# acids-ircam/RAVE

Measured on NVIDIA H100. Metric: audio-seconds/s (v2 train step fwd+bwd, 48 kHz), higher is better.
Workload: dtype bf16

## Files before the change

### include/rave_b200.h

```cpp
#ifndef RAVE_B200_H
#define RAVE_B200_H

#include <stddef.h>
#include <stdint.h>

#ifdef __cplusplus
extern "C" {
#endif

#define RAVE_ACT_NONE 0
#define RAVE_ACT_LEAKY 1
#define RAVE_ACT_SNAKE 2

#define RAVE_PREC_FP32 0
#define RAVE_PREC_BF16 1
#define RAVE_PREC_TF32 2

int rave_b200_version(void);
const char *rave_b200_last_error(void);
unsigned long long rave_b200_launch_count(void);

int rave_pqmf_analysis_fwd(const float *x, const float *taps, float *y, int B, int T, int Lout,
                           int ntaps, int pad_l, int flip_sign, void *stream);
int rave_pqmf_synthesis_fwd(const float *x, const float *w, float *out, int B, int L, int K,
                            int pad_l, float scale, int flip_sign, void *stream);
int rave_pqmf_analysis_fast(const float *x, const float *Ct, const float *Qt, float *y, int B, int T, int Lout,
                            int pad_l, int flip_sign, void *stream);
int rave_pqmf_synthesis_fast(const float *x, const float *Cc, const float *Qt, float *out, int B, int L,
                             int pad_l, float scale, int flip_sign, void *stream);

int rave_conv1d_gather_f32(const float *src, const float *w, const float *bias, const float *res,
                           float *out, int B, int Cs, int Ls, int Cm, int Lo, int K, int stride,
                           int dil, int pad_l, long ws_m, long ws_c, int act, float slope,
                           const float *alpha, int post_act, float post_slope, const float *post_x,
                           const float *post_alpha, void *stream);
int rave_conv1d_scatter_f32(const float *src, const float *w, const float *bias, const float *res,
                            float *out, int B, int Cs, int Ls, int Cm, int Lo, int K, int stride,
                            int dil, int pad_l, long ws_m, long ws_c, int act, float slope,
                            const float *alpha, int post_act, float post_slope, const float *post_x,
                            const float *post_alpha, void *stream);

size_t rave_conv1d_wgrad_workspace_bytes(int B, int Ca, int Cc, int Lp, int K);
int rave_conv1d_wgrad_f32(const float *P, const float *Q, float *dw, int B, int Ca, int Lp, int Cc,
                          int Lq, int K, int stride, int dil, int pad_l, long os_a, long os_c,
                          int act_p, int act_q, float slope, const float *alpha, void *workspace,
                          void *stream);

int rave_weight_norm_fwd(const float *v, const float *g, float *w, float *norm_out, int C0, int R,
                         void *stream);
int rave_weight_norm_bwd(const float *dw, const float *v, const float *g, const float *norm,
                         float *dv, float *dg, int C0, int R, void *stream);

int rave_act_fwd(const float *x, float *y, int B, int C, int L, int act, float slope,
                 const float *alpha, void *stream);
int rave_act_bwd(const float *dy, const float *x, float *dx, float *dalpha, int B, int C, int L,
                 int act, float slope, const float *alpha, void *stream);
int rave_am_tanh_fwd(const float *x, float *y, int B, int C, int L, void *stream);
int rave_am_tanh_bwd(const float *dy, const float *x, float *dx, int B, int C, int L, void *stream);
int rave_reparam_fwd(const float *z, const float *eps, float *zs, float *kl_sum, int B, int C, int L, void *stream);
int rave_mmd_fwd(const float *z, const float *prior, float *means, float *mmd, int B, int D, int L, void *stream);
int rave_mmd_bwd(const float *z, const float *prior, const float *g, float *dz, int B, int D, int L, void *stream);
int rave_sphere_norm_fwd(const float *z, float *out, float *norm, int B, int C, int L, void *stream);
int  rave_latent_moments(const float *z, int B, int C, int L, int D, double *state, double *work, void *stream);
long rave_latent_moments_workspace_bytes(int B, int L, int D);
int rave_sphere_norm_bwd(const float *g, const float *out, const float *norm, float *dz, int B, int C, int L,
                         void *stream);

int rave_conv1d_tc_supported(int Cin, int Cout, int K, int stride, int dil);
int rave_dilated_unit_tc_supported(int C, int L);
int rave_dilated_unit_tc_fwd(const void *xa_bf16, const void *w3t_bf16, const void *w1t_bf16, void *a1_out,
                             float *out_f32, void *out_act, int B, int C, int L, int pitch, int dil, int pad_l,
                             float slope_in, float slope_mid, int act_out, float slope_out, void *stream);
int rave_conv1d_tc_plan(int B, int Cin, int Cout, int Lout, int K);
int rave_conv1d_tc_pp_stages(int B, int Cin, int Cout, int Lout, int K, int fm, int res_bf16);
int rave_conv1d_tc_pp_fwd_stages(int B, int Cin, int Cout, int Lout, int K);
int rave_conv1d_tc_wide_stages(int B, int Cin, int Cout, int Lout, int K);
int rave_conv1d_tc_fwd(const void *xa_bf16, const void *wt_bf16, const float *bias, const float *res,
                       const void *res_bf16, const void *dact_src_bf16, const void *res_act_bf16, float res_slope,
                       float *out_f32, void *out_act_bf16,
                       int B, int Cin, int Lin, int in_pitch, int Cout, int Lout,
                       int K, int stride, int dil, int pad_l, int act, float slope, int out_rows,
                       int out_row_stride, int out_row_offset, const float *fm_d, int fm_bh, void *stream);
int rave_conv1d_tc_fwd_x3(const void *xa_bf16, const void *wt_bf16, const float *bias, const float *res,
                          const void *res_act, float res_slope, float *out_f32, void *out_act, int B, int Cin, int Lin,
                          int in_pitch, int Cout, int Lout, int K, int stride, int dil, int pad_l, int act, float slope,
                          int out_rows, int out_row_stride, int out_row_offset, int act_cs, void *stream);
int rave_conv1d_tc_wgrad_splits(int B, int Cm, int Lp, int Cn, int K);
int rave_conv1d_tc_wgrad_plan(int B, int Cm, int Lp, int Cn, int K);
int rave_time_stack_cl(const float *x, void *out_bf16, int B, int C, int T, int F, int Fp, int Cp, int kt, int pt,
                       void *stream);
int rave_time_stack_cl_bwd(const void *g_bf16, float *gx, int B, int C, int T, int F, int Fp, int Cp, int kt, int pt,
                           void *stream);
int rave_time_stack_nhwc(const float *x, void *out_bf16, int B, int C, int T, int F, long sb, long st, int Fp, int Cp, int kt,
                         int pt, void *stream);
int rave_time_stack_nhwc_bwd(const void *g_bf16, float *gx, int B, int C, int T, int F, int Fp, int Cp, int kt, int pt,
                             void *stream);
int rave_time_stack_nhwc_dil(const float *x, void *out_bf16, int B, int C, int T, int F, long sb, long st, int Fp, int Cp,
                             int kt, int pt, int dil, void *stream);
int rave_time_stack_nhwc_dil_bwd(const void *g_bf16, float *gx, int B, int C, int T, int F, int Fp, int Cp, int kt, int pt,
                                 int dil, void *stream);
int rave_l1_stats_f32(const float *t, const float *v, float *stats, long n, void *stream);
int rave_l1_grad_f32(const float *t, const float *v, const float *d, float *gt, float *gv, long n, void *stream);
int rave_leaky_fm_fwd(const float *x, float *a, float *stats, long H, float slope, void *stream);
int rave_leaky_fm_bwd(const float *a, const float *g, const float *d, float *gx, long H, float slope, void *stream);
int rave_leaky_fm_stack_fwd(const float *x, float *a, float *stats, void *xs_bf16, long Rh, int T, int F, int C, int Fp,
                            float slope, void *stream);
int rave_leaky_fm_stack_bwd(const float *a, const void *gxs_bf16, const float *ga, const float *d, float *gx, long Rh, int T,
                            int F, int C, int Fp, float slope, void *stream);
int rave_leaky_fm_stack_dil_fwd(const float *x, float *a, float *stats, void *xs_bf16, long Rh, int T, int F, int C, int Fp,
                                int dil, float slope, void *stream);
int rave_leaky_fm_stack_dil_bwd(const float *a, const void *gxs_bf16, const float *ga, const float *d, float *gx, long Rh,
                                int T, int F, int C, int Fp, int dil, float slope, void *stream);
int rave_snake_cl_fwd(const void *h_bf16, const float *alpha, void *a_bf16, long rows, int C, void *stream);
int rave_snake_cl_bwd(const void *ga_bf16, const void *h_bf16, const float *alpha, const void *add_bf16, void *gh_bf16,
                      float *dalpha, long rows, int C, void *stream);
int rave_adain_cl_stats(const void *h_bf16, int B, int L, int pitch, int C, float *mean_x, float *std_x, float *mean_y,
                        float *std_y, const float *learn_x, const float *learn_y, float *num_update_x,
                        float *num_update_y, int max_batch, float *scale, float *shift, void *stream);
int rave_adain_snake_cl_fwd(void *h_bf16, const float *alpha, const float *scale, const float *shift, void *a_bf16,
                            int B, int L, int pitch, int C, void *stream);
int rave_conv1d_tc_wgrad(const void *P_bf16, const void *Q_bf16, float *dwt, float *dbias, int B, int Cm, int Lp,
                         int p_pitch, int Cn, int Lq, int q_pitch, int K, int stride, int dil, int pad_l,
                         void *stream);
int rave_tapmajor_to_weight_f32(const float *dwt, float *dw, int Cm, int Cn, int K, int transpose, int splits,
                                void *stream);
int rave_conv1d_c1_fwd(const float *x, const float *w, const float *bias, float *out_f32, void *out_act_bf16,
                       int R, int x_pitch, int Lin, int Cout, int Lout, int out_pitch, int K, int stride,
                       int pad_l, int act, float slope, void *stream);
int rave_conv1d_c1_wgrad_splits(int R, int Lout);
// ... 116 lines not shown
```

### rave_b200/_lib.py

```python
import ctypes
import os
from ctypes import c_float, c_int, c_long, c_longlong, c_size_t, c_ulonglong, c_void_p, c_char_p

_HERE = os.path.dirname(os.path.abspath(__file__))
LIB_PATH = os.path.join(_HERE, "csrc", "librave_b200.so")

_P, _I, _F, _L = c_void_p, c_int, c_float, c_long

SIGNATURES = {
    "rave_b200_version": (c_int, []),
    "rave_b200_last_error": (c_char_p, []),
    "rave_b200_launch_count": (c_ulonglong, []),
    "rave_pqmf_analysis_fwd": (c_int, [_P, _P, _P, _I, _I, _I, _I, _I, _I, _P]),
    "rave_pqmf_synthesis_fwd": (c_int, [_P, _P, _P, _I, _I, _I, _I, _F, _I, _P]),
    "rave_pqmf_analysis_fast": (c_int, [_P, _P, _P, _P, _I, _I, _I, _I, _I, _P]),
    "rave_pqmf_synthesis_fast": (c_int, [_P, _P, _P, _P, _I, _I, _I, _F, _I, _P]),
    "rave_conv1d_gather_f32": (c_int, [_P, _P, _P, _P, _P, _I, _I, _I, _I, _I, _I, _I, _I, _I, _L, _L,
                                       _I, _F, _P, _I, _F, _P, _P, _P]),
    "rave_conv1d_scatter_f32": (c_int, [_P, _P, _P, _P, _P, _I, _I, _I, _I, _I, _I, _I, _I, _I, _L, _L,
                                        _I, _F, _P, _I, _F, _P, _P, _P]),
    "rave_conv1d_wgrad_workspace_bytes": (c_size_t, [_I, _I, _I, _I, _I]),
    "rave_conv1d_wgrad_f32": (c_int, [_P, _P, _P, _I, _I, _I, _I, _I, _I, _I, _I, _I, _L, _L, _I, _I,
                                      _F, _P, _P, _P]),
    "rave_weight_norm_fwd": (c_int, [_P, _P, _P, _P, _I, _I, _P]),
    "rave_weight_norm_bwd": (c_int, [_P, _P, _P, _P, _P, _P, _I, _I, _P]),
    "rave_act_fwd": (c_int, [_P, _P, _I, _I, _I, _I, _F, _P, _P]),
    "rave_act_bwd": (c_int, [_P, _P, _P, _P, _I, _I, _I, _I, _F, _P, _P]),
    "rave_am_tanh_fwd": (c_int, [_P, _P, _I, _I, _I, _P]),
    "rave_am_tanh_bwd": (c_int, [_P, _P, _P, _I, _I, _I, _P]),
    "rave_reparam_fwd": (c_int, [_P, _P, _P, _P, _I, _I, _I, _P]),
    "rave_mmd_fwd": (c_int, [_P, _P, _P, _P, _I, _I, _I, _P]),
    "rave_mmd_bwd": (c_int, [_P, _P, _P, _P, _I, _I, _I, _P]),
    "rave_sphere_norm_fwd": (c_int, [_P, _P, _P, _I, _I, _I, _P]),
    "rave_sphere_norm_bwd": (c_int, [_P, _P, _P, _P, _I, _I, _I, _P]),
    "rave_latent_moments": (c_int, [_P, _I, _I, _I, _I, _P, _P, _P]),
    "rave_latent_moments_workspace_bytes": (c_long, [_I, _I, _I]),
    "rave_conv1d_tc_supported": (c_int, [_I, _I, _I, _I, _I]),
    "rave_dilated_unit_tc_supported": (c_int, [_I, _I]),
    "rave_dilated_unit_tc_fwd": (c_int, [_P, _P, _P, _P, _P, _P, _I, _I, _I, _I, _I, _I, _F, _F, _I, _F, _P]),
    "rave_conv1d_tc_plan": (c_int, [_I, _I, _I, _I, _I]),
    "rave_conv1d_tc_pp_stages": (c_int, [_I, _I, _I, _I, _I, _I, _I]),
    "rave_conv1d_tc_pp_fwd_stages": (c_int, [_I, _I, _I, _I, _I]),
    "rave_conv1d_tc_wide_stages": (c_int, [_I, _I, _I, _I, _I]),
    "rave_conv1d_tc_fwd": (c_int, [_P, _P, _P, _P, _P, _P, _P, _F, _P, _P, _I, _I, _I, _I, _I, _I, _I, _I, _I, _I, _I,
                                   _F, _I, _I, _I, _P, _I, _P]),
    "rave_conv1d_tc_fwd_x3": (c_int, [_P, _P, _P, _P, _P, _F, _P, _P, _I, _I, _I, _I, _I, _I, _I, _I, _I, _I, _I, _F, _I,
                                      _I, _I, _I, _P]),
    "rave_weight_prep_tc_multi_x3": (c_int, [_I, _P, _P]),
    "rave_ncl_to_cl_x3": (c_int, [_P, _P, _I, _I, _I, _P]),
    "rave_conv1d_tc_wgrad": (c_int, [_P, _P, _P, _P, _I, _I, _I, _I, _I, _I, _I, _I, _I, _I, _I, _P]),
    "rave_tapmajor_to_weight_f32": (c_int, [_P, _P, _I, _I, _I, _I, _I, _P]),
    "rave_conv1d_tc_wgrad_splits": (c_int, [_I, _I, _I, _I, _I]),
    "rave_conv1d_tc_wgrad_plan": (c_int, [_I, _I, _I, _I, _I]),
    "rave_time_stack_cl": (c_int, [_P, _P, _I, _I, _I, _I, _I, _I, _I, _I, _P]),
    "rave_time_stack_cl_bwd": (c_int, [_P, _P, _I, _I, _I, _I, _I, _I, _I, _I, _P]),
    "rave_time_stack_nhwc": (c_int, [_P, _P, _I, _I, _I, _I, ctypes.c_long, ctypes.c_long, _I, _I, _I, _I, _P]),
    "rave_time_stack_nhwc_bwd": (c_int, [_P, _P, _I, _I, _I, _I, _I, _I, _I, _I, _P]),
    "rave_time_stack_nhwc_dil": (c_int, [_P, _P, _I, _I, _I, _I, ctypes.c_long, ctypes.c_long, _I, _I, _I, _I, _I, _P]),
    "rave_time_stack_nhwc_dil_bwd": (c_int, [_P, _P, _I, _I, _I, _I, _I, _I, _I, _I, _I, _P]),
    "rave_l1_stats_f32": (c_int, [_P, _P, _P, ctypes.c_long, _P]),
    "rave_leaky_fm_fwd": (c_int, [_P, _P, _P, ctypes.c_long, ctypes.c_float, _P]),
    "rave_leaky_fm_bwd": (c_int, [_P, _P, _P, _P, ctypes.c_long, ctypes.c_float, _P]),
    "rave_leaky_fm_stack_fwd": (c_int, [_P, _P, _P, _P, ctypes.c_long, _I, _I, _I, _I, ctypes.c_float, _P]),
    "rave_leaky_fm_stack_bwd": (c_int, [_P, _P, _P, _P, _P, ctypes.c_long, _I, _I, _I, _I, ctypes.c_float, _P]),
    "rave_leaky_fm_stack_dil_fwd": (c_int, [_P, _P, _P, _P, ctypes.c_long, _I, _I, _I, _I, _I, ctypes.c_float, _P]),
    "rave_leaky_fm_stack_dil_bwd": (c_int, [_P, _P, _P, _P, _P, ctypes.c_long, _I, _I, _I, _I, _I, ctypes.c_float, _P]),
    "rave_l1_grad_f32": (c_int, [_P, _P, _P, _P, _P, ctypes.c_long, _P]),
    "rave_snake_cl_fwd": (c_int, [_P, _P, _P, ctypes.c_long, _I, _P]),
    "rave_snake_cl_bwd": (c_int, [_P, _P, _P, _P, _P, _P, ctypes.c_long, _I, _P]),
    "rave_adain_cl_stats": (c_int, [_P, _I, _I, _I, _I, _P, _P, _P, _P, _P, _P, _P, _P, _I, _P, _P, _P]),
    "rave_adain_snake_cl_fwd": (c_int, [_P, _P, _P, _P, _P, _I, _I, _I, _I, _P]),
    "rave_weight_prep_tc": (c_int, [_P, _P, _P, _P, _P, _I, _P, _P, _I, _I, _I, _I, _I, _I, _P]),
    "rave_weight_norm_bwd_tapmajor": (c_int, [_P, _P, _P, _P, _P, _P, _I, _I, _I, _I, _I, _I, _P]),
    "rave_conv1d_c1_fwd": (c_int, [_P, _P, _P, _P, _P, _I, _I, _I, _I, _I, _I, _I, _I, _I, _I, _F, _P]),
    "rave_conv1d_c1_wgrad_splits": (c_int, [_I, _I]),
    "rave_conv1d_c1_wgrad": (c_int, [_P, _P, _P, _I, _I, _I, _I, _I, _I, _I, _I, _I, _I, _P]),
    "rave_conv1d_c1_dgrad": (c_int, [_P, _P, _P, _I, _I, _I, _I, _I, _I, _I, _I, _I, _I, _P]),
    "rave_colsum_bf16": (c_int, [_P, _P, _I, _I, _I, _I, _I, _P]),
    "rave_im2col_c1": (c_int, [_P, _P, _I, _I, _I, _I, _I, _I, _I, _I, _I, _I, _I, _P]),
    "rave_gather_c1": (c_int, [_P, _P, _I, _I, _I, _I, _I, _I, _I, _I, _I, _I, _I, _P]),
    "rave_im2col_cin": (c_int, [_P, _P, _I, _I, _I, _I, _I, _I, _I, _I, _I, _I, _I, _I, _I, _P]),
    "rave_gather_cin": (c_int, [_P, _P, _I, _I, _I, _I, _I, _I, _I, _I, _I, _I, _I, _I, _I, _P]),
    "rave_fm_stats": (c_int, [_P, _P, _I, _I, _I, _I, _F, _P]),
    "rave_fm_grad": (c_int, [_P, _P, _P, _I, _I, _I, _I, _F, _P]),
    "rave_score_stats": (c_int, [_P, _P, _I, _I, _I, _I, _P]),
    "rave_score_grad": (c_int, [_P, _P, _P, _I, _I, _I, _I, _P]),
    "rave_spectral_stats": (c_int, [_P, _P, _P, _L, _F, _P]),
    "rave_spectral_grad": (c_int, [_P, _P, _P, _P, _P, _L, _F, _P]),
    "rave_stft_frames": (c_int, [_P, _P, _P, _I, _I, _I, _I, _P]),
    "rave_stft_frames_bwd": (c_int, [_P, _P, _P, _I, _I, _I, _I, _P]),
    "rave_stft_frames_valid": (c_int, [_P, _P, _P, _I, _I, _I, _I, _F, _P]),
    "rave_stft_frames_valid_bwd": (c_int, [_P, _P, _P, _I, _I, _I, _I, _F, _P]),
    "rave_rfft_bwd_scale": (c_int, [_P, _P, _L, _I, _I, _L, _L, _L, _P]),
    "rave_mel_log1p_fwd": (c_int, [_P, _P, _P, _P, _I, _I, _I, _I, _I, _F, _P]),
    "rave_mel_log1p_bwd": (c_int, [_P, _P, _P, _P, _P, _I, _I, _I, _I, _I, _F, _P]),
    "rave_gru_fwd": (c_int, [_P, _P, _P, _P, _P, _I, _I, _I, _P]),
# ... 107 lines not shown
```

### rave_b200/csrc/conv_tc.cu

```cuda
#include <string.h>

#include <type_traits>

#include "common.cuh"
#include "tc_common.cuh"

namespace rave {
namespace tc {

constexpr int BLOCK_M = 128;
constexpr int NUM_THREADS = 288;
constexpr int SMEM_MAX = 227 * 1024;

struct TcParams {
  int B, Cin, Lin, Cout, Lout, K, stride, dil, pad_l;
  int BL, BB;
  int n_lt, n_bg, n_nt;
  int num_kb;
  int act;
  float slope;
  const float *bias;
  const float *res;
  const __nv_bfloat16 *res_bf16;
  const __nv_bfloat16 *dact_src;
// ... 371 lines not shown
    for (int tile = blockIdx.x; tile < num_tiles; tile += gridDim.x, ++it) {
      const int prev = mma_mainloop<BLOCK_N, BLOCK_K, X3>(d, smem_base, ring, kblocks, lane);
      mma_drain<BLOCK_N>(d, ring, prev, lane);
      const int buf = p.nacc == 2 ? (it & 1) : 0;
      const uint32_t use = p.nacc == 2 ? (it >> 1) : it;
      mbar_wait(&tempty_bar[buf], (use & 1) ^ 1);
      acc_store<BLOCK_N>(d, threadIdx.x, 0, 128 * buf);
      mbar_arrive(&tfull_bar[buf]);
    }
  } else {
    constexpr int BOXC = L::OUT_BOXC;
    const int quad = warp & 3;
    const int row = quad * 32 + lane;
    const bool issuer = threadIdx.x == 160;
    int it = 0;
    for (int tile = blockIdx.x; tile < num_tiles; tile += gridDim.x, ++it) {
      const TileCoord t = tile_coord<BLOCK_N>(tile, p);
      const int n0 = t.n0;
      const int b = t.b0 + row / p.BL;
      const int l = t.l0 + row % p.BL;
      const bool valid = (b < p.B) && (l < p.Lout);
      const size_t orow = (size_t)b * p.out_rows + (size_t)l * p.out_row_stride + p.out_row_offset;

      const int buf = p.nacc == 2 ? (it & 1) : 0;
      const uint32_t use = p.nacc == 2 ? (it >> 1) : it;
      if (stg) {
        if (issuer) bulk_wait_read<0>();
        named_bar_sync(1, 128);
      }
      mbar_wait(&tfull_bar[buf], use & 1);
      const uint32_t taddr = (uint32_t)(128 * buf + quad * 32) << 16;
      tc_epilogue<BLOCK_N, X3, BOXC>(p, taddr, n0, valid, orow, p.fm_d ? (b < p.fm_bh ? 1 : -1) : 0, stg, row);
      __syncwarp();
      if (lane == 0) mbar_arrive(&tempty_bar[buf]);
      if (stg) {
        fence_proxy_async();
        named_bar_sync(1, 128);
        if (issuer) {
#pragma unroll
          for (int c = 0; c < BLOCK_N; c += BOXC)
            tma_store_3d(&tmap_o, stg + (c / BOXC) * (BLOCK_M * L::OUT_SPAN), n0 + c, t.l0, t.b0);
          bulk_commit();
        }
      }
    }
    if (stg && issuer) bulk_wait_all();
  }
}

constexpr int PP_THREADS = 384;

enum PpEpi : int { PP_FM = 1, PP_RS = 2, PP_FWD = 4, PP_BIAS = 8, PP_LEAKY = 16 };

template <int BLOCK_N, int BOXC, bool FM, bool RS>
__device__ __forceinline__ void pp_epilogue(float (*d)[BLOCK_N / 2], uint8_t *slot, const TcParams &p, int w, int lane,
                                            int b0) {
  constexpr int TILE_BYTES = BLOCK_M * BLOCK_N * 2;
  uint8_t *part = slot + TILE_BYTES;
  uint8_t *skip = slot + (FM ? 2 : 1) * TILE_BYTES;
  constexpr int SPAN = BOXC * 2, JB = BOXC / 8;
  const float d0 = FM ? __ldg(p.fm_d) : 0.f, d1 = FM ? __ldg(p.fm_d + 1) : 0.f;
  const uint32_t base = stg_offset<BOXC>(16 * w + (lane >> 2), 0) + 4 * (lane & 3);
#pragma unroll
  for (int h = 0; h < 2; ++h) {
#pragma unroll
    for (int r = 0; r < 2; ++r) {
      const int row = 64 * h + 16 * w + (lane >> 2) + 8 * r;
      const float d1r = (FM && b0 + row / p.BL < p.fm_bh) ? d1 : 0.f;
#pragma unroll
      for (int j = 0; j < BLOCK_N / 8; ++j) {
        const uint32_t off = (base ^ (uint32_t)((j % JB) << 4)) + (j / JB) * (BLOCK_M * SPAN) + (64 * h + 8 * r) * SPAN;
        float v0 = d[h][4 * j + 2 * r], v1 = d[h][4 * j + 2 * r + 1];
        const uint32_t dm = *reinterpret_cast<const uint32_t *>(slot + off);
        lrelu_mask(v0, v1, dm, p.slope);
        if (FM) fm_grad(v0, v1, dm, *reinterpret_cast<const uint32_t *>(part + off), d0, d1r);
        if (RS) add_bf16_pair(v0, v1, *reinterpret_cast<const uint32_t *>(skip + off));
        __nv_bfloat162 o = __floats2bfloat162_rn(v0, v1);
        *reinterpret_cast<uint32_t *>(slot + off) = *reinterpret_cast<uint32_t *>(&o);
      }
    }
  }
}

template <int BLOCK_N, int BOXC, bool BIAS, bool LEAKY, int NH = 2>
__device__ __forceinline__ void pp_fwd_epilogue(float (*d)[BLOCK_N / 2], uint8_t *slot, const TcParams &p, int w,
                                                int lane, int n0, int h0 = 0) {
  constexpr int SPAN = BOXC * 2, JB = BOXC / 8;
  const uint32_t base = stg_offset<BOXC>(16 * w + (lane >> 2), 0) + 4 * (lane & 3);
  const uint32_t sslot = smem_u32(slot);
  const float2 *bias = reinterpret_cast<const float2 *>(p.bias + n0 + 2 * (lane & 3));
#pragma unroll
  for (int j = 0; j < BLOCK_N / 8; ++j) {
    const float2 bb = BIAS ? __ldg(bias + 4 * j) : make_float2(0.f, 0.f);
    const uint32_t col = (base ^ (uint32_t)((j % JB) << 4)) + (j / JB) * (BLOCK_M * SPAN);
#pragma unroll
    for (int h = 0; h < NH; ++h) {
#pragma unroll
      for (int r = 0; r < 2; ++r) {
        float v0 = d[h][4 * j + 2 * r], v1 = d[h][4 * j + 2 * r + 1];
        if (BIAS) {
          v0 += bb.x;
          v1 += bb.y;
        }
        if (LEAKY) {
          v0 = fmaxf(v0, v0 * p.slope);
          v1 = fmaxf(v1, v1 * p.slope);
        }
        __nv_bfloat162 o = __floats2bfloat162_rn(v0, v1);
        asm volatile("st.shared.b32 [%0], %1;" ::"r"(sslot + col + (64 * (h0 + h) + 8 * r) * SPAN),
                     "r"(*reinterpret_cast<uint32_t *>(&o))
                     : "memory");
      }
    }
  }
}

template <int BLOCK_N, int BLOCK_K, int E>
__device__ __forceinline__ void conv_tc_pp_body(const CUtensorMap *tmap_a, const CUtensorMap *tmap_b,
                                                const CUtensorMap *tmap_m, const CUtensorMap *tmap_p,
                                                const CUtensorMap *tmap_r, const CUtensorMap *tmap_o,
                                                const TcParams &p) {
  using L = SmemLayout<BLOCK_N, BLOCK_K, false>;
  constexpr int BOXC = L::OUT_BOXC;
  constexpr int BOX_BYTES = BLOCK_M * L::OUT_SPAN;
// ... 169 lines not shown
      mbar_init(&empty_bar[s], 8);
    }
    mbar_init(oempty_bar, 1);
    fence_barrier_init();
  }
  __syncthreads();
  griddep_launch_dependents();
  griddep_wait();

  Ring ring{full_bar, empty_bar, STAGES, 0, 0};
  if (wg == 0) {
    warpgroup_reg_dealloc<56>();
    if (warp != 0) return;
    for (int tile = blockIdx.x; tile < num_tiles; tile += gridDim.x) {
      const TileCoord t = tile_coord<BLOCK_N>(tile, p);
      for (int k = 0; k < p.K; ++k) {
        const TapOrigin o = tap_origin(k, p.dil, p.pad_l, p.stride);
        for (int kb = 0; kb < p.num_kb; ++kb)
          produce_kblock<BLOCK_N, BLOCK_K, false>(smem, ring, &tmap_a, &tmap_b, p, t, o, k, kb);
      }
    }
  } else {
    warpgroup_reg_alloc<224>();
    const int h = wg - 1;
    const int w = warp & 3;
    const bool issuer = threadIdx.x == 128;
    const uint32_t smem_base = smem_u32(smem);
    uint8_t *slot = smem + p.ops_off;
    float d[1][BLOCK_N / 2];
    int u = 0;
    for (int tile = blockIdx.x; tile < num_tiles; tile += gridDim.x, ++u) {
      const int prev = mma_mainloop<BLOCK_N, BLOCK_K, false, 1>(d, smem_base, ring, kblocks, lane, h);
      mma_drain<BLOCK_N, 1>(d, ring, prev, lane);
      const TileCoord t = tile_coord<BLOCK_N>(tile, p);
      if (issuer && u > 0) {
        bulk_wait_read<0>();
        mbar_arrive(oempty_bar);
      }
      mbar_wait(oempty_bar, (u & 1) ^ 1);
      pp_fwd_epilogue<BLOCK_N, BOXC, BIAS, LEAKY, 1>(d, slot, p, w, lane, t.n0, h);
      fence_proxy_async();
      named_bar_sync(1, 256);
      if (issuer) {
#pragma unroll
        for (int cb = 0; cb < BLOCK_N / BOXC; ++cb)
          tma_store_3d(&tmap_o, slot + cb * BOX_BYTES, t.n0 + cb * BOXC, t.l0, t.b0);
        bulk_commit();
      }
    }
    if (issuer) bulk_wait_all();
  }
}

static CUtensorMapSwizzle swizzle_enum(int bytes) {
  return bytes == 128 ? CU_TENSOR_MAP_SWIZZLE_128B : bytes == 64 ? CU_TENSOR_MAP_SWIZZLE_64B
                                                                 : CU_TENSOR_MAP_SWIZZLE_32B;
}

static int pick_block_k(int Cin) {
  if (Cin % 64 == 0) return 64;
  if (Cin % 32 == 0) return 32;
  if (Cin % 16 == 0) return 16;
  return 0;
}

static int pick_block_n(int Cout, long m_tiles) {
  const int cands[] = {128, 96, 64, 48, 32, 16};
  constexpr int NC = sizeof(cands) / sizeof(cands[0]);
  int best = 0;
  for (int c : cands) {
    if (Cout % c) continue;
    if (!best) best = c;
    if (m_tiles * (Cout / c) >= 132) return c;
  }
  for (int i = NC - 1; i >= 0; --i)
    if (Cout % cands[i] == 0 && cands[i] >= 32) return cands[i];
  return best;
}

struct TcGeometry {
  int BK, BL, BB, n_lt, n_bg, BN, n_nt, num_kb;
};
static TcGeometry tc_geometry(int B, int Cin, int Cout, int Lout) {
  TcGeometry g;
  g.BK = pick_block_k(Cin);
  g.BL = 128;
  while (g.BL > Lout && g.BL > 8) g.BL >>= 1;
  g.BB = 128 / g.BL;
  g.n_lt = ceil_div(Lout, g.BL);
  g.n_bg = ceil_div(B, g.BB);
  g.BN = pick_block_n(Cout, (long)g.n_lt * g.n_bg);
  g.n_nt = g.BN ? Cout / g.BN : 0;
  g.num_kb = g.BK ? ceil_div(Cin, g.BK) : 0;
  return g;
}

template <int BK, typename F>
static int visit_block_n(int BN, F &f) {
  using std::integral_constant;
  switch (BN) {
    case 128: return f(integral_constant<int, BK>(), integral_constant<int, 128>());
    case 96: return f(integral_constant<int, BK>(), integral_constant<int, 96>());
    case 64: return f(integral_constant<int, BK>(), integral_constant<int, 64>());
    case 48: return f(integral_constant<int, BK>(), integral_constant<int, 48>());
    case 32: return f(integral_constant<int, BK>(), integral_constant<int, 32>());
    case 16: return f(integral_constant<int, BK>(), integral_constant<int, 16>());
  }
  set_error("conv1d_tc: no kernel for BLOCK_N=%d", BN);
  return 1;
}
template <typename F>
static int visit_tile(int BK, int BN, F &&f) {
  switch (BK) {
    case 64: return visit_block_n<64>(BN, f);
    case 32: return visit_block_n<32>(BN, f);
    case 16: return visit_block_n<16>(BN, f);
  }
  set_error("conv1d_tc: no kernel for BLOCK_K=%d", BK);
  return 1;
}

template <int BN>
static int encode_rows_map(CUtensorMap *m, const __nv_bfloat16 *base, const TcParams &p, int box_b) {
  using L = SmemLayout<BN, 64, false>;
  const cuuint64_t dims[3] = {(cuuint64_t)p.Cout, (cuuint64_t)p.Lout, (cuuint64_t)p.B};
  const cuuint64_t strides[2] = {(cuuint64_t)p.Cout * 2 * p.out_row_stride, (cuuint64_t)p.Cout * 2 * p.out_rows};
  const cuuint32_t box[3] = {(cuuint32_t)L::OUT_BOXC, (cuuint32_t)p.BL, (cuuint32_t)box_b};
  const CUresult r = encode_bf16_map(m, 3, base + (size_t)p.out_row_offset * p.Cout, dims, strides, box,
                                     swizzle_enum(L::OUT_SPAN), CU_TENSOR_MAP_L2_PROMOTION_NONE);
  if (r != CUDA_SUCCESS) {
    set_error("conv1d_tc: bf16 row tensor map encode failed (%d)", (int)r);
    return 1;
  }
  return 0;
}

template <int BN, int BK, bool FWD>
constexpr bool pp_built = FWD || !(BN == 96 && BK == 64);

template <int BN, int BK, bool FWD>
constexpr int pp_stages(int nops) {
  using L = SmemLayout<BN, BK, false>;
  if (!pp_built<BN, BK, FWD>) return 0;
  const int s = (SMEM_MAX - L::FIXED - 2 * nops * BLOCK_M * BN * 2) / L::STAGE_BYTES;
  return s < 2 ? 0 : s > 8 ? 8 : s;
}

template <int BN, int BK>
static int pp_fwd_stages(int kblocks) {
  const int s = pp_stages<BN, BK, true>(1);
  TcParams q;
  plan_smem<BN, BK, false>(kblocks, q);
  return s >= q.stages && (BN == 128 || kblocks <= 24) ? s : 0;
}

static int wide_block_k(int Cin) { return pick_block_k(Cin); }
template <int BK>
constexpr int wide_ring_stages() {
  using L = SmemLayout<WIDE_N, BK, false>;
  const int s = (SMEM_MAX - L::FIXED - L::STG_BYTES) / L::STAGE_BYTES;
  return s > 8 ? 8 : s;
}
constexpr int WIDE_MIN_KBLOCKS = 12;
static int wide_stages(int Cin, int Cout, int K) {
  const int BK = wide_block_k(Cin);
  if (BK < 32 || Cout % WIDE_N || K * ceil_div(Cin, BK) < WIDE_MIN_KBLOCKS) return 0;
  return BK == 64 ? wide_ring_stages<64>() : wide_ring_stages<32>();
}

template <int BK>
static int launch_wide(const CUtensorMap &ta, const CUtensorMap &tb, TcParams p, int stages, cudaStream_t stream) {
  using L = SmemLayout<WIDE_N, BK, false>;
  p.stages = stages;
  p.ops_bytes = L::STG_BYTES;
  p.ops_off = p.stages * L::STAGE_BYTES;
  p.bar_off = p.ops_off + p.ops_bytes;
  const int grid = persistent_grid(p.n_lt * p.n_bg * p.n_nt), smem = p.bar_off + L::FIXED;
  CUtensorMap to;
  if (encode_rows_map<WIDE_N>(&to, p.out_act, p, p.BB)) return 1;
  const auto go = [&](auto bias, auto leaky) {
    return launch_tc<conv_tc_wide_kernel<BK, decltype(bias)::value, decltype(leaky)::value>>(
        "conv1d_tc", grid, PP_THREADS, smem, stream, ta, tb, to, p);
  };
  const std::true_type y;
  const std::false_type n;
  const bool leaky = p.act == RAVE_ACT_LEAKY;
  return p.bias ? (leaky ? go(y, y) : go(y, n)) : (leaky ? go(n, y) : go(n, n));
}

template <int BN, int BK, bool FWD>
static int launch_pp(const CUtensorMap &ta, const CUtensorMap &tb, TcParams p, int stages, cudaStream_t stream) {
  using L = SmemLayout<BN, BK, false>;
  p.stages = stages;
  p.ops_bytes = (1 + (p.fm_d ? 1 : 0) + (p.res_bf16 ? 1 : 0)) * BLOCK_M * BN * 2;
  p.ops_off = p.stages * L::STAGE_BYTES;
  p.bar_off = p.ops_off + 2 * p.ops_bytes;
  const int grid = persistent_grid(p.n_lt * p.n_bg * p.n_nt), smem = p.bar_off + L::FIXED;
  const std::true_type y;
  const std::false_type n;
  CUtensorMap tm, tp, tr, to;
  if (encode_rows_map<BN>(&to, p.out_act, p, p.BB)) return 1;
  if constexpr (FWD) {
    const auto go = [&](auto bias, auto leaky) {
      return launch_tc<conv_tc_pp_fwd_kernel<BN, BK, decltype(bias)::value, decltype(leaky)::value>>(
          "conv1d_tc", grid, PP_THREADS, smem, stream, ta, tb, to, p);
    };
    const bool leaky = p.act == RAVE_ACT_LEAKY;
    return p.bias ? (leaky ? go(y, y) : go(y, n)) : (leaky ? go(n, y) : go(n, n));
  } else {
    memset(&tp, 0, sizeof(tp));
    memset(&tr, 0, sizeof(tr));
    if (encode_rows_map<BN>(&tm, p.dact_src, p, p.BB)) return 1;
    if (p.fm_d && encode_rows_map<BN>(&tp, p.fm_bh > 0 ? p.dact_src : p.dact_src - p.fm_half, p, 1)) return 1;
    if (p.res_bf16 && encode_rows_map<BN>(&tr, p.res_bf16, p, p.BB)) return 1;
    const auto go = [&](auto fm, auto rs) {
      return launch_tc<conv_tc_pp_kernel<BN, BK, decltype(fm)::value, decltype(rs)::value>>(
          "conv1d_tc", grid, PP_THREADS, smem, stream, ta, tb, tm, tp, tr, to, p);
    };
    return p.fm_d ? (p.res_bf16 ? go(y, y) : go(y, n)) : (p.res_bf16 ? go(n, y) : go(n, n));
  }
}

template <int BN, int BK, bool X3>
static int launch(const CUtensorMap &ta, const CUtensorMap &tb, TcParams p, cudaStream_t stream) {
  using L = SmemLayout<BN, BK, X3>;
  plan_smem<BN, BK, X3>(p.K * p.num_kb, p);
  if (!p.out_act) p.stg = 0;
  CUtensorMap to;
  memset(&to, 0, sizeof(to));
  if (p.stg && encode_rows_map<BN>(&to, p.out_act, p, p.BB)) return 1;
  return launch_tc<conv_tc_kernel<BN, BK, X3>>("conv1d_tc", persistent_grid(p.n_lt * p.n_bg * p.n_nt), NUM_THREADS,
                                               p.bar_off + L::FIXED, stream, ta, tb, to, p);
}

int conv_tc_dispatch_x3(int BK, int BN, const CUtensorMap &ta, const CUtensorMap &tb, const TcParams &p, cudaStream_t s);
#ifdef RAVE_TC_X3_UNIT
int conv_tc_dispatch_x3(int BK, int BN, const CUtensorMap &ta, const CUtensorMap &tb, const TcParams &p, cudaStream_t s) {
  return visit_tile(BK, BN, [&](auto bk, auto bn) {
    return launch<decltype(bn)::value, decltype(bk)::value, true>(ta, tb, p, s);
  });
}
#endif

}
}

#ifndef RAVE_TC_X3_UNIT
extern "C" int rave_conv1d_tc_supported(int Cin, int Cout, int K, int stride, int dil) {
  if (rave::tc::pick_block_k(Cin) == 0) return 0;
  if (Cout % 16) return 0;
  if (K < 1 || stride < 1 || dil < 1) return 0;
  return 1;
}

extern "C" int rave_conv1d_tc_plan(int B, int Cin, int Cout, int Lout, int K) {
  using namespace rave::tc;
  const TcGeometry g = tc_geometry(B, Cin, Cout, Lout);
  if (!g.BK || !g.BN) return 0;
  TcParams q;
  visit_tile(g.BK, g.BN, [&](auto bk, auto bn) {
    plan_smem<decltype(bn)::value, decltype(bk)::value, false>(K * g.num_kb, q);
    return 0;
  });
  return g.BN | (g.BK << 12) | (q.nacc - 1) << 24 | q.stg << 25 | q.stages << 26;
}

extern "C" int rave_conv1d_tc_pp_stages(int B, int Cin, int Cout, int Lout, int K, int fm, int res_bf16) {
  using namespace rave::tc;
  const TcGeometry g = tc_geometry(B, Cin, Cout, Lout);
  if (!g.BK || !g.BN) return 0;
  const int nops = 1 + (fm ? 1 : 0) + (res_bf16 ? 1 : 0);
  return visit_tile(g.BK, g.BN, [&](auto bk, auto bn) {
    return pp_stages<decltype(bn)::value, decltype(bk)::value, false>(nops);
  });
}

extern "C" int rave_conv1d_tc_pp_fwd_stages(int B, int Cin, int Cout, int Lout, int K) {
  using namespace rave::tc;
  const TcGeometry g = tc_geometry(B, Cin, Cout, Lout);
  if (!g.BK || !g.BN) return 0;
  return visit_tile(g.BK, g.BN, [&](auto bk, auto bn) {
    return pp_fwd_stages<decltype(bn)::value, decltype(bk)::value>(K * g.num_kb);
  });
}

extern "C" int rave_conv1d_tc_wide_stages(int B, int Cin, int Cout, int Lout, int K) {
  using namespace rave::tc;
  const TcGeometry g = tc_geometry(B, Cin, Cout, Lout);
  if (!g.BK || !g.BN) return 0;
  return wide_stages(Cin, Cout, K);
}

static int conv1d_tc_fwd_impl(const void *xa, const void *wt, const float *bias, const float *res,
                              const void *res_bf16, const void *dact_src, const void *res_act, float res_slope,
                              float *out_f32, void *out_act,
                              int B, int Cin, int Lin, int in_pitch, int Cout, int Lout,
                              int K, int stride, int dil, int pad_l, int act, float slope, int out_rows,
                              int out_row_stride, int out_row_offset, const float *fm_d, int fm_bh,
                              void *stream, int x3, int act_cs = 0) {
  using namespace rave;
  using namespace rave::tc;
  RAVE_CHECK_ARG(!x3 || (!res_bf16 && !dact_src && !fm_d),
                 "conv1d_tc(x3): the split-operand mode has no gradient epilogues (forward path only)");
  RAVE_CHECK_ARG(xa && wt && (out_f32 || out_act), "conv1d_tc: null pointer");
  RAVE_CHECK_ARG(rave_conv1d_tc_supported(Cin, Cout, K, stride, dil), "conv1d_tc: unsupported shape Cin=%d Cout=%d",
                 Cin, Cout);
  if (in_pitch <= 0) in_pitch = Lin;
  RAVE_CHECK_ARG(in_pitch >= ceil_div(Lin, stride) * stride,
                 "conv1d_tc: input pitch %d < Lin %d rounded up to the stride %d (slack rows must be zero)", in_pitch,
                 Lin, stride);
  RAVE_CHECK_ARG(act == RAVE_ACT_NONE || act == RAVE_ACT_LEAKY, "conv1d_tc: epilogue activation %d unsupported", act);
  RAVE_CHECK_ARG(act != RAVE_ACT_LEAKY || (slope >= 0.f && slope <= 1.f), "conv1d_tc: LeakyReLU slope %g outside [0, 1]",
                 (double)slope);
  RAVE_CHECK_ARG(!res_act || (res_slope > 0.f && res_slope <= 1.f), "conv1d_tc: res_slope %g outside (0, 1]",
                 (double)res_slope);
  RAVE_CHECK_ARG(((uintptr_t)bias & 15) == 0, "conv1d_tc: bias must be 16-byte aligned");
  RAVE_CHECK_ARG(((uintptr_t)xa & 15) == 0 && ((uintptr_t)wt & 15) == 0, "conv1d_tc: operands must be 16B aligned");
  RAVE_CHECK_ARG((((uintptr_t)out_f32 | (uintptr_t)out_act | (uintptr_t)res | (uintptr_t)res_bf16 | (uintptr_t)dact_src |
                   (uintptr_t)res_act) & 31) == 0,
                 "conv1d_tc: epilogue tensors must be 32-byte aligned (256-bit row segments)");
  RAVE_CHECK_ARG(get_encode_fn(), "conv1d_tc: cuTensorMapEncodeTiled not available");

  const TcGeometry g = tc_geometry(B, Cin, Cout, Lout);
  RAVE_CHECK_ARG(g.BN > 0, "conv1d_tc: no BLOCK_N for Cout=%d", Cout);
  const bool bf16_only = out_act && !res && !res_act && !out_f32;
  const bool pp_dgrad = bf16_only && dact_src && !bias && act == RAVE_ACT_NONE;
  const bool pp_fwd = bf16_only && !dact_src && !res_bf16 && !fm_d;
  const int wide = !x3 && pp_fwd ? wide_stages(Cin, Cout, K) : 0;
  const int BK = wide ? wide_block_k(Cin) : g.BK, BN = wide ? WIDE_N : g.BN;
  const CUtensorMapL2promotion promo = BK == 64 ? CU_TENSOR_MAP_L2_PROMOTION_L2_256B : CU_TENSOR_MAP_L2_PROMOTION_NONE;
  TcParams p;
  p.B = B; p.Cin = Cin; p.Lin = Lin; p.Cout = Cout; p.Lout = Lout; p.K = K; p.stride = stride; p.dil = dil;
  p.pad_l = pad_l; p.act = act; p.slope = slope; p.bias = bias; p.res = res; p.out_f32 = out_f32;
  p.res_bf16 = (const __nv_bfloat16 *)res_bf16; p.dact_src = (const __nv_bfloat16 *)dact_src;
  p.res_act = (const __nv_bfloat16 *)res_act;
  p.res_inv_slope = (res_act && res_slope > 0.f) ? 1.f / res_slope : 1.f;
  p.out_act = (__nv_bfloat16 *)out_act;
  p.out_rows = out_rows > 0 ? out_rows : Lout;
  p.out_row_stride = out_row_stride > 0 ? out_row_stride : 1;
  p.out_row_offset = out_row_offset;
  RAVE_CHECK_ARG(!fm_d || (dact_src && slope > 0.f && ((fm_bh > 0 && 2 * fm_bh == B) || (fm_bh < 0 && -fm_bh == B))),
                 "conv1d_tc: the fused feature-matching gradient needs dact_src and a [real; fake] batch (B=%d, fm_bh=%d)",
                 B, fm_bh);
  p.fm_d = fm_d;
  p.fm_bh = fm_bh > 0 ? fm_bh : 0;
  p.fm_half = (long)(fm_bh > 0 ? fm_bh : -fm_bh) * p.out_rows * Cout;
  p.act_ld = x3 ? 2 * Cout : Cout;
  p.act_cs = act_cs > 0 ? act_cs : Cout;
  RAVE_CHECK_ARG(!x3 || (Cout % p.act_cs == 0 && p.act_cs % 16 == 0),
                 "conv1d_tc(x3): %d channels per position do not tile the %d-column rows in 16-column chunks", p.act_cs,
                 Cout);
  RAVE_CHECK_ARG(!x3 || !res_act || p.act_cs == Cout, "conv1d_tc(x3): res_act needs one position per row");
  p.BL = g.BL; p.BB = g.BB; p.n_lt = g.n_lt; p.n_bg = g.n_bg;
  p.n_nt = Cout / BN;
  p.num_kb = ceil_div(Cin, BK);

  CUtensorMap ta, tb;
  {
    const cuuint64_t ca = (cuuint64_t)Cin * (x3 ? 2 : 1);
    const cuuint64_t dims[4] = {ca, (cuuint64_t)stride, (cuuint64_t)ceil_div(Lin, stride), (cuuint64_t)B};
    const cuuint64_t strides[3] = {ca * 2, ca * 2 * stride, ca * 2 * in_pitch};
    const cuuint32_t box[4] = {(cuuint32_t)BK, 1, (cuuint32_t)p.BL, (cuuint32_t)p.BB};
    const CUresult r = encode_bf16_map(&ta, 4, xa, dims, strides, box, swizzle_enum(BK * 2), promo);
    RAVE_CHECK_ARG(r == CUDA_SUCCESS, "conv1d_tc: tensor map A encode failed (%d)", (int)r);
  }
  {
    const cuuint64_t dims[2] = {(cuuint64_t)Cin, (cuuint64_t)K * Cout * (x3 ? 2 : 1)};
    const cuuint64_t strides[1] = {(cuuint64_t)Cin * 2};
    const cuuint32_t box[2] = {(cuuint32_t)BK, (cuuint32_t)BN};
    const CUresult r = encode_bf16_map(&tb, 2, wt, dims, strides, box, swizzle_enum(BK * 2), promo);
    RAVE_CHECK_ARG(r == CUDA_SUCCESS, "conv1d_tc: tensor map B encode failed (%d)", (int)r);
  }
  cudaStream_t s = (cudaStream_t)stream;
  if (x3) return conv_tc_dispatch_x3(BK, BN, ta, tb, p, s);
  if (wide) return BK == 64 ? launch_wide<64>(ta, tb, p, wide, s) : launch_wide<32>(ta, tb, p, wide, s);
  const int nops = 1 + (fm_d ? 1 : 0) + (res_bf16 ? 1 : 0);
  return visit_tile(BK, BN, [&](auto bk, auto bn) {
    constexpr int BK_ = decltype(bk)::value, BN_ = decltype(bn)::value;
    if constexpr (pp_built<BN_, BK_, false>) {
      const int stages = pp_dgrad ? pp_stages<BN_, BK_, false>(nops) : 0;
      if (stages) return launch_pp<BN_, BK_, false>(ta, tb, p, stages, s);
    }
    if constexpr (pp_built<BN_, BK_, true>) {
      const int stages = pp_fwd ? pp_fwd_stages<BN_, BK_>(K * g.num_kb) : 0;
      if (stages) return launch_pp<BN_, BK_, true>(ta, tb, p, stages, s);
    }
    return launch<BN_, BK_, false>(ta, tb, p, s);
  });
}

extern "C" int rave_conv1d_tc_fwd(const void *xa, const void *wt, const float *bias, const float *res,
                                  const void *res_bf16, const void *dact_src, const void *res_act, float res_slope,
                                  float *out_f32, void *out_act,
                                  int B, int Cin, int Lin, int in_pitch, int Cout, int Lout,
                                  int K, int stride, int dil, int pad_l, int act, float slope, int out_rows,
                                  int out_row_stride, int out_row_offset, const float *fm_d, int fm_bh,
                                  void *stream) {
  return conv1d_tc_fwd_impl(xa, wt, bias, res, res_bf16, dact_src, res_act, res_slope, out_f32, out_act, B, Cin, Lin,
                            in_pitch, Cout, Lout, K, stride, dil, pad_l, act, slope, out_rows, out_row_stride,
                            out_row_offset, fm_d, fm_bh, stream, 0);
}

extern "C" int rave_conv1d_tc_fwd_x3(const void *xa, const void *wt, const float *bias, const float *res,
                                     const void *res_act, float res_slope, float *out_f32, void *out_act,
                                     int B, int Cin, int Lin, int in_pitch, int Cout, int Lout,
                                     int K, int stride, int dil, int pad_l, int act, float slope, int out_rows,
                                     int out_row_stride, int out_row_offset, int act_cs, void *stream) {
  return conv1d_tc_fwd_impl(xa, wt, bias, res, nullptr, nullptr, res_act, res_slope, out_f32, out_act, B, Cin, Lin,
                            in_pitch, Cout, Lout, K, stride, dil, pad_l, act, slope, out_rows, out_row_stride,
                            out_row_offset, nullptr, 0, stream, 1, act_cs);
}

namespace rave {
namespace tc {

constexpr int WG_ROWS = 64;
constexpr int WG_SLAB = WG_ROWS * 128;

struct WgParams {
  int B, Cm, Lp, Cn, Lq, K, stride, dil, pad_l;
  int BL, BB, n_lt, n_bg;
  int n_mt, n_nt, splits;
  float *dwt;
  float *dbias;
  float *dbias_part;
};

template <int BLOCK_N>
// ... 300 lines not shown
```

Baseline: 2474.

## Add wide-N persistent dgrad kernel with split-warpgroup epilogue for bf16 convs

Adds a persistent warp-specialized dgrad conv kernel that uses the wide N tile, with each of the two consumer warpgroups owning one 64-row half of the tile and running the leaky-mask and feature-matching epilogue on that half. It is chosen for bf16 dgrad convs with enough k-blocks and no bf16 residual. A new row-tiling helper picks the L-block size that minimises padded rows for the wide paths, and this also changes geometry for the existing wide forward kernel. The goal is more reuse of each A tile across output channels and fewer tiles for large convs, at the cost of more shared memory per stage and fewer pipeline stages.

```diff
diff --git a/include/rave_b200.h b/include/rave_b200.h
--- a/include/rave_b200.h
+++ b/include/rave_b200.h
@@ -75,6 +75,7 @@
 int rave_conv1d_tc_pp_stages(int B, int Cin, int Cout, int Lout, int K, int fm, int res_bf16);
 int rave_conv1d_tc_pp_fwd_stages(int B, int Cin, int Cout, int Lout, int K);
 int rave_conv1d_tc_wide_stages(int B, int Cin, int Cout, int Lout, int K);
+int rave_conv1d_tc_wide_dgrad_stages(int B, int Cin, int Cout, int Lout, int K, int fm, int res_bf16);
 int rave_conv1d_tc_fwd(const void *xa_bf16, const void *wt_bf16, const float *bias, const float *res,
                        const void *res_bf16, const void *dact_src_bf16, const void *res_act_bf16, float res_slope,
                        float *out_f32, void *out_act_bf16,
diff --git a/rave_b200/_lib.py b/rave_b200/_lib.py
--- a/rave_b200/_lib.py
+++ b/rave_b200/_lib.py
@@ -42,6 +42,7 @@
     "rave_conv1d_tc_pp_stages": (c_int, [_I, _I, _I, _I, _I, _I, _I]),
     "rave_conv1d_tc_pp_fwd_stages": (c_int, [_I, _I, _I, _I, _I]),
     "rave_conv1d_tc_wide_stages": (c_int, [_I, _I, _I, _I, _I]),
+    "rave_conv1d_tc_wide_dgrad_stages": (c_int, [_I, _I, _I, _I, _I, _I, _I]),
     "rave_conv1d_tc_fwd": (c_int, [_P, _P, _P, _P, _P, _P, _P, _F, _P, _P, _I, _I, _I, _I, _I, _I, _I, _I, _I, _I, _I,
                                    _F, _I, _I, _I, _P, _I, _P]),
     "rave_conv1d_tc_fwd_x3": (c_int, [_P, _P, _P, _P, _P, _F, _P, _P, _I, _I, _I, _I, _I, _I, _I, _I, _I, _I, _I, _F, _I,
diff --git a/rave_b200/csrc/conv_tc.cu b/rave_b200/csrc/conv_tc.cu
--- a/rave_b200/csrc/conv_tc.cu
+++ b/rave_b200/csrc/conv_tc.cu
@@ -447,9 +447,9 @@
 
 enum PpEpi : int { PP_FM = 1, PP_RS = 2, PP_FWD = 4, PP_BIAS = 8, PP_LEAKY = 16 };
 
-template <int BLOCK_N, int BOXC, bool FM, bool RS>
+template <int BLOCK_N, int BOXC, bool FM, bool RS, int NH = 2>
 __device__ __forceinline__ void pp_epilogue(float (*d)[BLOCK_N / 2], uint8_t *slot, const TcParams &p, int w, int lane,
-                                            int b0) {
+                                            int b0, int h0 = 0) {
   constexpr int TILE_BYTES = BLOCK_M * BLOCK_N * 2;
   uint8_t *part = slot + TILE_BYTES;
   uint8_t *skip = slot + (FM ? 2 : 1) * TILE_BYTES;
@@ -457,14 +457,15 @@
   const float d0 = FM ? __ldg(p.fm_d) : 0.f, d1 = FM ? __ldg(p.fm_d + 1) : 0.f;
   const uint32_t base = stg_offset<BOXC>(16 * w + (lane >> 2), 0) + 4 * (lane & 3);
 #pragma unroll
-  for (int h = 0; h < 2; ++h) {
+  for (int h = 0; h < NH; ++h) {
 #pragma unroll
     for (int r = 0; r < 2; ++r) {
-      const int row = 64 * h + 16 * w + (lane >> 2) + 8 * r;
+      const int row = 64 * (h0 + h) + 16 * w + (lane >> 2) + 8 * r;
       const float d1r = (FM && b0 + row / p.BL < p.fm_bh) ? d1 : 0.f;
 #pragma unroll
       for (int j = 0; j < BLOCK_N / 8; ++j) {
-        const uint32_t off = (base ^ (uint32_t)((j % JB) << 4)) + (j / JB) * (BLOCK_M * SPAN) + (64 * h + 8 * r) * SPAN;
+        const uint32_t off =
+            (base ^ (uint32_t)((j % JB) << 4)) + (j / JB) * (BLOCK_M * SPAN) + (64 * (h0 + h) + 8 * r) * SPAN;
         float v0 = d[h][4 * j + 2 * r], v1 = d[h][4 * j + 2 * r + 1];
         const uint32_t dm = *reinterpret_cast<const uint32_t *>(slot + off);
         lrelu_mask(v0, v1, dm, p.slope);
@@ -740,6 +741,107 @@
   }
 }
 
+template <int BLOCK_K, bool FM>
+__global__ void __launch_bounds__(PP_THREADS, 1)
+conv_tc_wide_dgrad_kernel(const __grid_constant__ CUtensorMap tmap_a, const __grid_constant__ CUtensorMap tmap_b,
+                          const __grid_constant__ CUtensorMap tmap_m, const __grid_constant__ CUtensorMap tmap_p,
+                          const __grid_constant__ CUtensorMap tmap_o, const TcParams p) {
+  constexpr int BLOCK_N = WIDE_N;
+  using L = SmemLayout<BLOCK_N, BLOCK_K, false>;
+  constexpr int BOXC = L::OUT_BOXC;
+  constexpr int BOX_BYTES = BLOCK_M * L::OUT_SPAN;
+  constexpr int TILE_BYTES = BLOCK_M * BLOCK_N * 2;
+  const int STAGES = p.stages;
+
+  extern __shared__ uint8_t smem_raw[];
+  uint8_t *smem = reinterpret_cast<uint8_t *>((reinterpret_cast<uintptr_t>(smem_raw) + 1023) & ~uintptr_t(1023));
+  uint64_t *full_bar = reinterpret_cast<uint64_t *>(smem + p.bar_off);
+  uint64_t *empty_bar = full_bar + STAGES;
+  uint64_t *ofull_bar = empty_bar + STAGES;
+  uint64_t *wfull_bar = ofull_bar + 1;
+  uint8_t *slot = smem + p.ops_off;
+
+  const int wg = threadIdx.x >> 7;
+  const int warp = threadIdx.x >> 5;
+  const int lane = threadIdx.x & 31;
+  const int num_tiles = p.n_lt * p.n_bg * p.n_nt;
+  const int kblocks = p.K * p.num_kb;
+
+  if (threadIdx.x == 0) {
+    tma_prefetch_desc(&tmap_a);
+    tma_prefetch_desc(&tmap_b);
+    tma_prefetch_desc(&tmap_m);
+    if constexpr (FM) tma_prefetch_desc(&tmap_p);
+    tma_prefetch_desc(&tmap_o);
+    for (int s = 0; s < STAGES; ++s) {
+      mbar_init(&full_bar[s], 1);
+      mbar_init(&empty_bar[s], 8);
+    }
+    mbar_init(ofull_bar, 1);
+    mbar_init(wfull_bar, 256);
+    fence_barrier_init();
+  }
+  __syncthreads();
+  griddep_launch_dependents();
+  griddep_wait();
+
+  Ring ring{full_bar, empty_bar, STAGES, 0, 0};
+  if (wg == 0) {
+    warpgroup_reg_dealloc<56>();
+    if (warp == 0) {
+      for (int tile = blockIdx.x; tile < num_tiles; tile += gridDim.x) {
+        const TileCoord t = tile_coord<BLOCK_N>(tile, p);
+        for (int k = 0; k < p.K; ++k) {
+          const TapOrigin o = tap_origin(k, p.dil, p.pad_l, p.stride);
+          for (int kb = 0; kb < p.num_kb; ++kb)
+            produce_kblock<BLOCK_N, BLOCK_K, false>(smem, ring, &tmap_a, &tmap_b, p, t, o, k, kb);
+        }
+      }
+    } else if (warp == 1 && lane == 0) {
+      int u = 0;
+      for (int tile = blockIdx.x; tile < num_tiles; tile += gridDim.x, ++u) {
+        const TileCoord t = tile_coord<BLOCK_N>(tile, p);
+        if (u > 0) bulk_wait_read<0>();
+        mbar_arrive_expect_tx(ofull_bar, p.ops_bytes);
+#pragma unroll
+        for (int cb = 0; cb < BLOCK_N / BOXC; ++cb) {
+          tma_load_3d(slot + cb * BOX_BYTES, &tmap_m, ofull_bar, t.n0 + cb * BOXC, t.l0, t.b0);
+          if (FM) {
+            for (int i = 0; i < p.BB; ++i) {
+              const int b = t.b0 + i;
+              const int pb = p.fm_bh > 0 ? (b < p.fm_bh ? b + p.fm_bh : b - p.fm_bh) : b;
+              tma_load_3d(slot + TILE_BYTES + cb * BOX_BYTES + i * p.BL * L::OUT_SPAN, &tmap_p, ofull_bar,
+                          t.n0 + cb * BOXC, t.l0, pb);
+            }
+          }
+        }
+        mbar_wait(wfull_bar, u & 1);
+#pragma unroll
+        for (int cb = 0; cb < BLOCK_N / BOXC; ++cb)
+          tma_store_3d(&tmap_o, slot + cb * BOX_BYTES, t.n0 + cb * BOXC, t.l0, t.b0);
+        bulk_commit();
+      }
+      bulk_wait_all();
+    }
+  } else {
+    warpgroup_reg_alloc<224>();
+    const int h = wg - 1;
+    const int w = warp & 3;
+    const uint32_t smem_base = smem_u32(smem);
+    float d[1][BLOCK_N / 2];
+    int u = 0;
+    for (int tile = blockIdx.x; tile < num_tiles; tile += gridDim.x, ++u) {
+      const int prev = mma_mainloop<BLOCK_N, BLOCK_K, false, 1>(d, smem_base, ring, kblocks, lane, h);
+      mma_drain<BLOCK_N, 1>(d, ring, prev, lane);
+      const TileCoord t = tile_coord<BLOCK_N>(tile, p);
+      mbar_wait(ofull_bar, u & 1);
+      pp_epilogue<BLOCK_N, BOXC, FM, false, 1>(d, slot, p, w, lane, t.b0, h);
+      fence_proxy_async();
+      mbar_arrive(wfull_bar);
+    }
+  }
+}
+
 static CUtensorMapSwizzle swizzle_enum(int bytes) {
   return bytes == 128 ? CU_TENSOR_MAP_SWIZZLE_128B : bytes == 64 ? CU_TENSOR_MAP_SWIZZLE_64B
                                                                  : CU_TENSOR_MAP_SWIZZLE_32B;
@@ -781,6 +883,20 @@
   g.n_nt = g.BN ? Cout / g.BN : 0;
   g.num_kb = g.BK ? ceil_div(Cin, g.BK) : 0;
   return g;
+}
+
+static void wide_rows(int B, int Lout, TcGeometry &g) {
+  long best = -1;
+  for (int bl = 128; bl >= 8; bl >>= 1) {
+    const long rows = (long)ceil_div(Lout, bl) * bl * ceil_div(B, 128 / bl) * (128 / bl);
+    if (best < 0 || rows < best) {
+      best = rows;
+      g.BL = bl;
+    }
+  }
+  g.BB = 128 / g.BL;
+  g.n_lt = ceil_div(Lout, g.BL);
+  g.n_bg = ceil_div(B, g.BB);
 }
 
 template <int BK, typename F>
@@ -874,6 +990,39 @@
   const std::false_type n;
   const bool leaky = p.act == RAVE_ACT_LEAKY;
   return p.bias ? (leaky ? go(y, y) : go(y, n)) : (leaky ? go(n, y) : go(n, n));
+}
+
+template <bool FM>
+constexpr int wide_dgrad_ring_stages() {
+  using L = SmemLayout<WIDE_N, 64, false>;
+  const int s = (SMEM_MAX - L::FIXED - (FM ? 2 : 1) * L::STG_BYTES) / L::STAGE_BYTES;
+  return s > 8 ? 8 : s;
+}
+constexpr int WIDE_DGRAD_MIN_KBLOCKS = 12, WIDE_DGRAD_MIN_KBLOCKS_FM = 24;
+static int wide_dgrad_stages(int Cin, int Cout, int K, bool fm, bool res_bf16) {
+  if (res_bf16 || Cin % 64 || Cout % WIDE_N) return 0;
+  if (K * (Cin / 64) < (fm ? WIDE_DGRAD_MIN_KBLOCKS_FM : WIDE_DGRAD_MIN_KBLOCKS)) return 0;
+  return fm ? wide_dgrad_ring_stages<true>() : wide_dgrad_ring_stages<false>();
+}
+
+static int launch_wide_dgrad(const CUtensorMap &ta, const CUtensorMap &tb, TcParams p, int stages,
+                             cudaStream_t stream) {
+  using L = SmemLayout<WIDE_N, 64, false>;
+  p.stages = stages;
+  p.ops_bytes = (p.fm_d ? 2 : 1) * L::STG_BYTES;
+  p.ops_off = p.stages * L::STAGE_BYTES;
+  p.bar_off = p.ops_off + p.ops_bytes;
+  const int grid = persistent_grid(p.n_lt * p.n_bg * p.n_nt), smem = p.bar_off + L::FIXED;
+  CUtensorMap tm, tp, to;
+  memset(&tp, 0, sizeof(tp));
+  if (encode_rows_map<WIDE_N>(&to, p.out_act, p, p.BB)) return 1;
+  if (encode_rows_map<WIDE_N>(&tm, p.dact_src, p, p.BB)) return 1;
+  if (p.fm_d && encode_rows_map<WIDE_N>(&tp, p.fm_bh > 0 ? p.dact_src : p.dact_src - p.fm_half, p, 1)) return 1;
+  if (p.fm_d)
+    return launch_tc<conv_tc_wide_dgrad_kernel<64, true>>("conv1d_tc", grid, PP_THREADS, smem, stream, ta, tb, tm, tp,
+                                                          to, p);
+  return launch_tc<conv_tc_wide_dgrad_kernel<64, false>>("conv1d_tc", grid, PP_THREADS, smem, stream, ta, tb, tm, tp,
+                                                         to, p);
 }
 
 template <int BN, int BK, bool FWD>
@@ -979,6 +1128,13 @@
   return wide_stages(Cin, Cout, K);
 }
 
+extern "C" int rave_conv1d_tc_wide_dgrad_stages(int B, int Cin, int Cout, int Lout, int K, int fm, int res_bf16) {
+  using namespace rave::tc;
+  const TcGeometry g = tc_geometry(B, Cin, Cout, Lout);
+  if (!g.BK || !g.BN) return 0;
+  return wide_dgrad_stages(Cin, Cout, K, fm != 0, res_bf16 != 0);
+}
+
 static int conv1d_tc_fwd_impl(const void *xa, const void *wt, const float *bias, const float *res,
                               const void *res_bf16, const void *dact_src, const void *res_act, float res_slope,
                               float *out_f32, void *out_act,
@@ -1015,7 +1171,8 @@
   const bool pp_dgrad = bf16_only && dact_src && !bias && act == RAVE_ACT_NONE;
   const bool pp_fwd = bf16_only && !dact_src && !res_bf16 && !fm_d;
   const int wide = !x3 && pp_fwd ? wide_stages(Cin, Cout, K) : 0;
-  const int BK = wide ? wide_block_k(Cin) : g.BK, BN = wide ? WIDE_N : g.BN;
+  const int wide_dgrad = !x3 && pp_dgrad ? wide_dgrad_stages(Cin, Cout, K, fm_d != nullptr, res_bf16 != nullptr) : 0;
+  const int BK = wide ? wide_block_k(Cin) : g.BK, BN = wide || wide_dgrad ? WIDE_N : g.BN;
   const CUtensorMapL2promotion promo = BK == 64 ? CU_TENSOR_MAP_L2_PROMOTION_L2_256B : CU_TENSOR_MAP_L2_PROMOTION_NONE;
   TcParams p;
   p.B = B; p.Cin = Cin; p.Lin = Lin; p.Cout = Cout; p.Lout = Lout; p.K = K; p.stride = stride; p.dil = dil;
@@ -1039,7 +1196,9 @@
                  "conv1d_tc(x3): %d channels per position do not tile the %d-column rows in 16-column chunks", p.act_cs,
                  Cout);
   RAVE_CHECK_ARG(!x3 || !res_act || p.act_cs == Cout, "conv1d_tc(x3): res_act needs one position per row");
-  p.BL = g.BL; p.BB = g.BB; p.n_lt = g.n_lt; p.n_bg = g.n_bg;
+  TcGeometry m = g;
+  if (wide || wide_dgrad) wide_rows(B, Lout, m);
+  p.BL = m.BL; p.BB = m.BB; p.n_lt = m.n_lt; p.n_bg = m.n_bg;
   p.n_nt = Cout / BN;
   p.num_kb = ceil_div(Cin, BK);
 
@@ -1062,6 +1221,7 @@
   cudaStream_t s = (cudaStream_t)stream;
   if (x3) return conv_tc_dispatch_x3(BK, BN, ta, tb, p, s);
   if (wide) return BK == 64 ? launch_wide<64>(ta, tb, p, wide, s) : launch_wide<32>(ta, tb, p, wide, s);
+  if (wide_dgrad) return launch_wide_dgrad(ta, tb, p, wide_dgrad, s);
   const int nops = 1 + (fm_d ? 1 : 0) + (res_bf16 ? 1 : 0);
   return visit_tile(BK, BN, [&](auto bk, auto bn) {
     constexpr int BK_ = decltype(bk)::value, BN_ = decltype(bn)::value;
```

After: 2565, median of 6. 1.04x the previous value.
